# ootts/EasyHeC

Measured on AMD Instinct MI355X. Metric: mask-render fwd+bwd frames/sec, xArm7 50k-tri @1280x720x8-view, higher is better.
Workload: dtype f32; 1 GPU; xarm7_1280x720_8view; robot=xarm7 (41096 tris, 20525 verts), views_per_gpu=8, global_views=8, links=8, antialias=True, optimizer=Adam lr 3e-3 wd 5e-4, ref_sums=bound once, mask_output=False, step=HIP launch chain, parallelism=single GPU

## Files before the change

easyhec_amd/csrc/ehr_fused_core.h:

```cpp
#pragma once
#include "ehr_host.h"
#include "ehr_pose_core.h"
#include "ehr_raster_core.h"

namespace ehr {

#define EHR_FIX_SCALE 4294967296.0
__device__ __forceinline__ long long fix_of(float v) { return __double2ll_rn((double)v * EHR_FIX_SCALE); }
__device__ __forceinline__ void fix_add(long long* acc, float v, int* meta) {
    if (!(fabsf(v) < 1.0e9f)) {
        atomicOr(&meta[EHR_META_OVERFLOW], 1);
        return;
    }
    if (v != 0.f) atomicAdd((unsigned long long*)acc, (unsigned long long)fix_of(v));
}
__device__ __forceinline__ void fix_add_delta(long long* acc, float v, long long cached, int* meta) {
    if (!(fabsf(v) < 1.0e9f)) {
        atomicOr(&meta[EHR_META_OVERFLOW], 1);
        return;
    }
    const long long d = ((v != 0.f) ? fix_of(v) : 0ll) - cached;
    if (d != 0) atomicAdd((unsigned long long*)acc, (unsigned long long)d);
}
__device__ __forceinline__ float fix_get(long long q) { return (float)((double)q * (1.0 / EHR_FIX_SCALE)); }
__device__ __forceinline__ long long acc_load(const long long* p) {
    return __hip_atomic_load(p, __ATOMIC_RELAXED, __HIP_MEMORY_SCOPE_AGENT);
}

__host__ __device__ constexpr int vb_acc_stride(int L, int nls = VB_LOSS_SLOTS) { return 12 * L + nls * VB_LOSS_STRIDE; }
__host__ __device__ __forceinline__ int* vb_acc_meta(long long* acc, int B, int L) { return (int*)(acc + (size_t)B * vb_acc_stride(L)); }

struct StepTail {
    const float* K;
    const float* link_poses;
    const float* tc_jac;
    float* red;
    float* dof;
    float* m;
    float* v;
    int* step;
    float* loss_out;
    float* grad_out;
    float n, f, lr, b1, b2, eps, wd;
    int defer_adam;
};

struct FinishPre {
    AdamState st;
    PoseBwdPre pb;
    long long vt;
};

template <bool TAIL>
__device__ __forceinline__ void finish_prefetch(FinishPre& pre, const BinGeom& g, int B, const long long* __restrict__ vtot,
                                                const StepTail& tail, int nls, float (*Js)[16] ,
                                                float* lp_lds ) {
    const int tid = threadIdx.x;
    if (TAIL && !tail.defer_adam) pre.st = pose_adam_fetch(tail.dof, tail.m, tail.v, tail.step);
    pre.vt = (nls == 32 && vtot && (tid & 31) == 0 && (tid >> 5) < B) ? vtot[tid >> 5] : 0ll;
    if (TAIL) {
        pose_backward_prefetch(pre.pb, tail.K, tail.link_poses, tail.tc_jac, B, g.L, g.H, g.W, tail.n, tail.f, Js, lp_lds);
        if (!tail.defer_adam) pose_adam_bias(pre.st, tail.lr, tail.b1, tail.b2);
    }
}

template <bool TAIL>
__device__ __forceinline__ void finish_reduce(const FinishPre& pre, const BinGeom& g, int B, const long long* __restrict__ facc,
                                              const long long* __restrict__ vtot, float* __restrict__ loss,
                                              float* __restrict__ grad_mvp, int* __restrict__ meta, const StepTail& tail,
                                              int nls, int lstride, double (*S)[17] ,
                                              float* red_lds , float (*Js)[16] ,
                                              const float* lp_lds ) {
    const int tid = threadIdx.x, L = g.L;
    const int acc_stride = vb_acc_stride(L, nls);
    auto view_loss_slow = [&](int b) {
// ... 120 lines not shown
```

easyhec_amd/csrc/ehr_host.h:

```cpp
#pragma once
#include <hip/hip_runtime.h>
#include <stdint.h>
#include <stdio.h>

#include <string>
#include <vector>

#include "../../include/ehr.h"

struct ehr_ctx;

namespace ehr {

void set_error(const std::string& msg);
int fail(int code, const char* fmt, ...);

#define EHR_HIP(call)                                                                                   \
    do {                                                                                                \
        hipError_t e_ = (call);                                                                         \
        if (e_ != hipSuccess)                                                                           \
            return ::ehr::fail(EHR_ERR_HIP, "%s failed: %s (%s:%d)", #call, hipGetErrorString(e_), __FILE__, __LINE__); \
    } while (0)

#define EHR_LAUNCH_CHECK()                                                                              \
// ... 30 lines not shown
int vbuf_plan(ehr_ctx* ctx, int B, int L, int V, int T, int H, int W, float slack, const float* verts,
              const int32_t* tris, const int32_t* tri_link, const int32_t* opp);
int vbuf_meta_read(ehr_ctx* ctx, int* meta4);
int vbuf_bind_ref(ehr_ctx* ctx, const float* ref, int views, hipStream_t stream);
int vbuf_score(ehr_ctx* ctx, const float* verts, const int32_t* tris, const int32_t* vert_link, const float* mvp, int Q, int S,
               int L, int V, int T, int H, int W, long long* score, unsigned char* count, hipStream_t stream, int* handled);
int vbuf_overlap(ehr_ctx* ctx, const float* verts, const int32_t* tris, const int32_t* vert_link, const float* mvp,
                 const float* ref, int Q, int S, int L, int V, int T, int H, int W, long long* overlap, long long* ref_area,
                 hipStream_t stream, int* handled);
int vbuf_chain(ehr_ctx* ctx, const float* verts, const int32_t* tris, const int32_t* vert_link,
               const int32_t* opp, float* mvp, const float* ref, int B, int L, int V, int T, int H, int W, float* mask,
               float* loss, float* grad_mvp, const StepHead* head, const StepTail* tail, hipStream_t stream,
               int multi_views = 0);

}

struct ehr_ctx {
    int device = 0;
    ehr::Scratch counts;
    unsigned long long counts_clean = ~0ull;
    bool vb_slow_needed = false;
    ehr::Scratch ranges;
    std::vector<int32_t> ranges_last;
    unsigned long long ranges_moves = ~0ull;
    ehr::Scratch rkeys;
    unsigned long long rkeys_clean = ~0ull;
    ehr::Scratch offsets;
    ehr::Scratch entries;
    size_t entries_cap = 0;
    int* host_pinned = nullptr;
    hipEvent_t ev_size[2] = {nullptr, nullptr};
    bool size_valid[2] = {false, false};
    ehr::RasterShape size_shape[2] = {};
    int size_slot = 0;
    int pB = 0, pL = 0, pV = 0, pT = 0, pH = 0, pW = 0;
    int num_cus = 256;
    ehr::Scratch vb_clus;
    ehr::Scratch vb_heavy;
    ehr::Scratch vb_idx;
    const void* vb_plan_tris = nullptr;
    const void* vb_plan_opp = nullptr;
    const void* vb_plan_verts = nullptr;
    int vb_nc = 0;
    int vb_jcap = 0;
    int vb_chunk = 0;
    ehr::Scratch vb_boxes;
    ehr::Scratch vb_units;
    ehr::Scratch vb_acc;
    ehr::Scratch vb_posc;
    bool vb_lazy = false;
    ehr::Scratch vb_jobs;
    ehr::Scratch vb_spill;
    int vb_spill_cap = 0;
    ehr::Scratch vb_refsum;
    const float* vb_ref = nullptr;
    int vb_ref_views = 0;
    const float* vb_weight = nullptr;
    int vb_weight_views = 0;
    ehr::Scratch vb_hstate;
    ehr::Scratch vb_hstate_m;
    ehr::Scratch sc_counts, sc_offsets, sc_entries, sc_posc;
    ehr::Scratch sc_img;
    size_t sc_entries_cap = 0;
    ehr::Scratch sc_clus, sc_misc;
    int sc_nc = 0;
    const void* sc_key[3] = {nullptr, nullptr, nullptr};
    int sc_key_n[3] = {0, 0, 0};
    unsigned long long sc_hash = 0;
    bool sc_mixed = false;
    void* comm = nullptr;
    int comm_ranks = 0;
    void* p2p_mail = nullptr;
    void* p2p_peer[EHR_P2P_MAX_RANKS] = {};
    int p2p_ranks = 0, p2p_rank = 0;
    hipStream_t cap_stream = nullptr;
    hipGraphExec_t gexec = nullptr;
    unsigned long long gexec_reallocs = 0;
    unsigned long long scratch_moves() const {
        unsigned long long n = 0;
        for (const ehr::Scratch* s : {&counts, &offsets, &entries, &vb_clus, &vb_heavy, &vb_idx, &vb_boxes, &vb_units, &vb_acc,
                                      &vb_posc, &vb_jobs, &vb_spill, &vb_refsum, &vb_hstate, &vb_hstate_m, &sc_counts, &sc_offsets, &sc_entries, &sc_posc, &sc_clus, &sc_misc, &sc_img})
            n += s->moves;
        return n;
    }
    bool capturing = false;
    bool timing = false;
    std::vector<hipEvent_t> ev;
    size_t ev_used = 0;
};
```

easyhec_amd/csrc/ehr_vbuf.hip:

```cpp
#include <stdlib.h>
#include <string.h>

#include <algorithm>
#include <utility>
#include <vector>

#include "ehr_fused_core.h"

namespace ehr {

constexpr int VB_RW = EHR_TILE_W + 2;
constexpr int VB_RH = EHR_TILE_H + 2;
constexpr int VB_RN = VB_RW * VB_RH;
constexpr int VB_WORDS = (VB_RN + 63) / 64;
constexpr int VB_LBOX_STRIDE = 16;
constexpr int VB_HEAVY_T_DEFAULT = 3000;
constexpr int VB_HEAVY_CAP = 4096;
constexpr int VB_MED_CAP = 2048;
constexpr int VB_MED_T_DEFAULT = 1500;
constexpr int VB_PRIO_LONG = 3;
constexpr int VB_PRIO_HEAVY = 2;
constexpr int VB_JOB_ITEMS = 64;
constexpr int VB_SPILL_BLOCK = 2048;
constexpr u64 VB_EMPTY = ~0ull;
// ... 1445 lines not shown
        for (int j = 0; j < 4; j++)
            if (ix + j < W) mask[im + j] = 0.f;
    }
}

struct VbCompArgs {
    const long long* tsum;
    int nls, want_grad, vec_ok;
    float* loss;
    int B;
    long long* facc;
    int do_finish, B_all;
    const float* mvp;
    int spill_cap;
    int* lbox_all;
    VbSlots sl;
    float* mask;
    const float* verts;
    const float* ref;
    const long long* vtot_all;
    int* meta;
    float* grad_mvp;
    const VbItem* spill;
    int V;
    const long long* facc_all;
    const int* ref_flag;
    BinGeom g;
};

struct VbSharedRef {
    int view0, nviews;
};
struct VbWeight {
    const float* w;
    int view0, nviews;
};
struct VbCompParamsW;
typedef const VbCompParamsW __attribute__((address_space(4)))* VbCompParamsWPtr;
__device__ __forceinline__ VbCompParamsWPtr vb_comp_params_w();
__device__ __forceinline__ VbWeight vb_comp_weight(VbCompParamsWPtr p);
__device__ __forceinline__ void vb_read_weights(const VbWeight& wt, int b, int H, int W, int row, int ix, const bool* pin, int vec_ok, float* wf) {
    const size_t imw = ((size_t)((wt.view0 + b) % wt.nviews) * H + row) * W + ix;
    if (vec_ok) {
        if (pin[0]) {
            const float4 w4 = *reinterpret_cast<const float4*>(wt.w + imw);
            wf[0] = w4.x; wf[1] = w4.y; wf[2] = w4.z; wf[3] = w4.w;
        }
    } else {
#pragma unroll
        for (int j = 0; j < 4; j++)
            if (pin[j]) wf[j] = wt.w[imw + j];
    }
}
template <bool FILL, bool SHARED = false, bool WEIGHTED = false>
__device__ __forceinline__ void vb_composite_items(const VbCompArgs& C, const int* s_jbase, const unsigned* s_utile, float* gpix,
                                                   int xcd, int wslot, int nslots, int nwg, VbSharedRef sh = {0, 1}) {
    const BinGeom& g = C.g;
    const int lane = lane_id(), wave = (int)(threadIdx.x >> 6);
    const int W = g.W, H = g.H, L = g.L, B = C.B, U = B * L;
    const bool sparse = C.tsum != nullptr;
    const int jcap = C.sl.jcap, nls = C.nls, want_grad = C.want_grad, vec_ok = C.vec_ok, V = C.V, spill_cap = C.spill_cap;
    const float *const mvpc = C.mvp, *const verts = C.verts, *const jval = C.sl.jval, *const ref = C.ref;
    const int *const jn = C.sl.jn, *const jspill = C.sl.jspill;
    const VbItem *const jitems = C.sl.jitems, *const spill = C.spill;
    float* const mask = C.mask;
    long long* const facc = C.facc;
    int* const meta = C.meta;
    const long long* const tsum = C.tsum;
    const int nitems = sparse ? min(s_jbase[U], jcap) : B * g.nt;
    const int per_xcd = vb_xcd_share(nitems);
    const int ibeg = xcd * per_xcd, iend = min(ibeg + per_xcd, nitems);
    const int istep = nslots;
    const int acc_stride = vb_acc_stride(L, nls);
    const int r = lane >> 3, c4 = (lane & 7) * 4;
    const float invL = __builtin_amdgcn_rcpf((float)L);
    const VbCompParamsWPtr wparams = vb_comp_params_w();
    for (int item = ibeg + wslot; item < iend; item += istep) {
    int b, tx, ty;
    if (sparse) {
        int lo = 0;
        if (U <= 64) {
            lo = __popcll(__ballot(lane < U && s_jbase[lane] <= item)) - 1;
        } else {
            int hi = U - 1;
            while (lo < hi) {
                const int mid = (lo + hi + 1) >> 1;
                if (s_jbase[mid] <= item)
                    lo = mid;
                else
                    hi = mid - 1;
            }
        }
        b = vb_div_small(lo, invL);
        const unsigned ut = s_utile[lo];
        const int nx = (int)(ut >> 22), k = item - s_jbase[lo];
        const int kr = vb_div_small(k, __builtin_amdgcn_rcpf((float)nx));
        ty = (int)((ut >> 10) & 4095u) + kr;
        tx = (int)(ut & 1023u) + k - kr * nx;
        bool prior = false;
        if (lane < lo - b * L) {
            const int u2 = b * L + lane;
            const unsigned u2t = s_utile[u2];
            const int n2 = s_jbase[u2 + 1] - s_jbase[u2];
            const int ax0 = u2t & 1023u, ay0 = (u2t >> 10) & 4095u, anx = u2t >> 22;
            prior = n2 > 0 && tx >= ax0 && tx < ax0 + anx && ty >= ay0 && (ty - ay0) * anx < n2;
        }
        if (__ballot(prior)) continue;
    } else {
        b = item / g.nt;
        const int tile = item - b * g.nt;
        tx = tile % g.ntx;
        ty = tile / g.ntx;
    }
    const int tile = ty * g.ntx + tx;
    long long* const vacc = facc + (size_t)b * acc_stride;
    long long* const lacc = vacc + 12 * L + (tile % nls) * VB_LOSS_STRIDE;
    const int rx0 = tx * EHR_TILE_W - 1, ry0 = ty * EHR_TILE_H - 1;
    unsigned tmask;
    int myn = -1, myslot = 0;
    {
        if (lane < L) {
            const int u = b * L + lane;
            const unsigned ut = s_utile[u];
            const int j0 = s_jbase[u], n = s_jbase[u + 1] - j0;
            const int tx0 = ut & 1023u, ty0 = (ut >> 10) & 4095u, nx = ut >> 22;
            if (n > 0 && tx >= tx0 && tx < tx0 + nx && ty >= ty0 && (ty - ty0) * nx < n) {
                myslot = j0 + (ty - ty0) * nx + (tx - tx0);
                if (myslot < jcap) myn = jn[myslot];
            }
        }
        tmask = (unsigned)__ballot(myn >= 0);
    }
    if (sparse && tmask == 0) {
        if (FILL) {
            const int zx = tx * EHR_TILE_W + c4, zy = ty * EHR_TILE_H + r;
            vb_zero_tile_row(mask, ((size_t)b * H + (H - 1 - (zy < H ? zy : 0))) * W + zx, zy < H, zx, W, vec_ok);
        }
        continue;
    }
    const int ix = tx * EHR_TILE_W + c4, iy = ty * EHR_TILE_H + r;
    const bool row_in = iy < H;
    const size_t im = ((size_t)b * H + (H - 1 - (row_in ? iy : 0))) * W + ix;
    const size_t imr = SHARED ? ((size_t)((sh.view0 + b) % sh.nviews) * H + (H - 1 - (row_in ? iy : 0))) * W + ix : im;
    float rf[4] = {0.f, 0.f, 0.f, 0.f};
    bool pin[4];
#pragma unroll
    for (int j = 0; j < 4; j++) pin[j] = row_in && (ix + j) < W;
    if (vec_ok) {
        if (pin[0]) {
            const float4 r4 = *reinterpret_cast<const float4*>(ref + imr);
            rf[0] = r4.x; rf[1] = r4.y; rf[2] = r4.z; rf[3] = r4.w;
        }
    } else {
#pragma unroll
        for (int j = 0; j < 4; j++)
            if (pin[j]) rf[j] = ref[imr + j];
    }
    float wf[4] = {0.f, 0.f, 0.f, 0.f};
    if (WEIGHTED) vb_read_weights(vb_comp_weight(wparams), b, H, W, H - 1 - (row_in ? iy : 0), ix, pin, vec_ok, wf);
    float acc[4] = {0.f, 0.f, 0.f, 0.f};
    unsigned todo = tmask;
    while (todo) {
        const int l = __ffs(todo) - 1;
        todo &= todo - 1;
        const size_t slot = (size_t)vb_readlane(myslot, l);
        const float4 v4 = *reinterpret_cast<const float4*>(jval + slot * 256 + r * EHR_TILE_W + c4);
        acc[0] += v4.x;
        acc[1] += v4.y;
        acc[2] += v4.z;
        acc[3] += v4.w;
    }
    float e2 = 0.f, gv[4];
    float mv[4];
#pragma unroll
    for (int j = 0; j < 4; j++) {
        gv[j] = 0.f;
        mv[j] = 0.f;
        if (pin[j]) {
            const float m = acc[j] > 1.f ? 1.f : acc[j];
            const float e = m - rf[j];
            if (WEIGHTED) {
                const float we = wf[j] * e;
                e2 += we * e;
                gv[j] = (acc[j] <= 1.f) ? 2.f * we : 0.f;
            } else {
                e2 += e * e;
                gv[j] = (acc[j] <= 1.f) ? 2.f * e : 0.f;
            }
            mv[j] = m;
        }
    }
    if (mask) {
        if (vec_ok) {
            if (pin[0]) *reinterpret_cast<float4*>(mask + im) = make_float4(mv[0], mv[1], mv[2], mv[3]);
        } else {
#pragma unroll
            for (int j = 0; j < 4; j++)
                if (pin[j]) mask[im + j] = mv[j];
        }
    }
    {
        const float s = wave_sum(e2);
        if (lane == 0) {
            if (sparse)
                fix_add_delta(lacc, s, tsum[(size_t)b * g.nt + tile], meta);
            else
                fix_add(lacc, s, meta);
        }
    }
    const unsigned bmask = (unsigned)__ballot(myn > 0);
    if (!want_grad || bmask == 0) continue;

    VB_WAVE_SYNC();
#pragma unroll
    for (int j = 0; j < 4; j++) gpix[r * EHR_TILE_W + c4 + j] = gv[j];
    VB_WAVE_SYNC();
    unsigned links = bmask;
    while (links) {
        const int l = __ffs(links) - 1;
        links &= links - 1;
        const size_t slot = (size_t)vb_readlane(myslot, l);
        int n = vb_readlane(myn, l);
        int sbase = 0;
        if (n > VB_JOB_ITEMS) {
            sbase = jspill[slot];
            if (sbase < 0 || sbase >= spill_cap) n = VB_JOB_ITEMS;
            else n = min(n, VB_JOB_ITEMS + (spill_cap - sbase));
        }
        const VbVertsT<true> pv = vb_verts<true>(VbLazy{verts, mvpc + ((size_t)b * L + l) * 16, nullptr});
        float G[12];
#pragma unroll
        for (int k = 0; k < 12; k++) G[k] = 0.f;
        for (int i = lane; i < n; i += 64) {
            const VbItem itm = *((i < VB_JOB_ITEMS) ? &jitems[slot * VB_JOB_ITEMS + i] : &spill[sbase + (i - VB_JOB_ITEMS)]);
            const int q = itm.packed & 1023, d = (itm.packed >> 10) & 1;
            const int tri1 = (itm.packed >> 13) & 1;
            const float dc = ((itm.packed >> 14) & 1) ? 1.f : -1.f;
            const int nq = q + (d ? VB_RW : 1);
            const int oq = (itm.alpha > 0.f) ? q : nq;
            const int oy = vb_div_rw(oq), ox = oq - oy * VB_RW;
            const float gi = gpix[(oy - 1) * EHR_TILE_W + (ox - 1)];
            const float dd = gi * dc;
            if (gi == 0.f || dd == 0.f) continue;
            const int qy = vb_div_rw(q), qx = q - qy * VB_RW;
            int px = rx0 + qx, py = ry0 + qy;
            if (tri1) {
                px += 1 - d;
                py += d;
            }
            float g1[3], g2[3];
            const float* a1 = verts + 3 * (size_t)itm.v1;
            const float* a2 = verts + 3 * (size_t)itm.v2;
            const float h1[4] = {a1[0], a1[1], a1[2], 1.f}, h2[4] = {a2[0], a2[1], a2[2], 1.f};
            aa_pos_grad(transform_vertex(pv.M, h1[0], h1[1], h1[2]), transform_vertex(pv.M, h2[0], h2[1], h2[2]), px, py, d,
                        itm.alpha, dd, W, H, g1, g2);
#pragma unroll
            for (int rr = 0; rr < 3; rr++)
#pragma unroll
                for (int c = 0; c < 4; c++) G[4 * rr + c] += g1[rr] * h1[c] + g2[rr] * h2[c];
        }
        const float mine = wave_sum12(G, lane);
        if ((lane & 3) == 0 && (lane & 12) != 12) fix_add(&vacc[12 * l + wave_sum12_element(lane)], mine, meta);
    }
    }
    if (FILL) {
        const int total = B * g.nt;
        for (int t = (int)blockIdx.x * 4 + wave; t < total; t += nwg * 4) {
            const int b = t / g.nt, tile = t - b * g.nt;
            const int ty = tile / g.ntx, tx = tile - ty * g.ntx;
            bool owned = false;
            if (lane < L) {
                const int u = b * L + lane;
                const unsigned ut = s_utile[u];
                const int n = s_jbase[u + 1] - s_jbase[u];
                const int tx0 = ut & 1023u, ty0 = (ut >> 10) & 4095u, nx = ut >> 22;
                owned = n > 0 && tx >= tx0 && tx < tx0 + nx && ty >= ty0 && (ty - ty0) * nx < n;
            }
            if (__ballot(owned)) continue;
            const int ix = tx * EHR_TILE_W + c4, iy = ty * EHR_TILE_H + r;
            const bool row_in = iy < H;
            vb_zero_tile_row(mask, ((size_t)b * H + (H - 1 - (row_in ? iy : 0))) * W + ix, row_in, ix, W, vec_ok);
        }
    }
}

constexpr int VB_JOB_WAVES = 4;
struct VbCoverOut {
    u64* tcov;
    int* sticky;
    int S;
};
struct VbJobParams {
    BinGeom g;
    int B;
    VbClusters cl;
    VbRecs rc;
    const int* lbox;
    int use_hint;
    VbHeavy hv;
    VbSlotIdx si;
    int heavy_t, med_t0;
    VbResolveArgs rq;
    VbCoverOut co;
};
typedef const VbJobParams __attribute__((address_space(4)))* VbJobParamsPtr;
__device__ __forceinline__ VbJobParamsPtr vb_job_params() {
    VbJobParamsPtr p = (VbJobParamsPtr)__builtin_amdgcn_kernarg_segment_ptr();
    asm volatile("" : "+s"(p));
    return p;
}
template <class T>
__device__ __forceinline__ T vb_prm_copy(const T __attribute__((address_space(4)))* p) {
    return *(const T*)p;
}
template <bool COVER, bool LAZY = false>
// ... 343 lines not shown
    const int r = lane >> 3, c4 = (lane & 7) * 4;
    const int ix = tx * EHR_TILE_W + c4, iy = ty * EHR_TILE_H + r;
    const bool row_in = iy < H;
    const size_t im = ((size_t)b * H + (H - 1 - (row_in ? iy : 0))) * W + ix;
    float rf[4] = {0.f, 0.f, 0.f, 0.f};
    bool pin[4];
#pragma unroll
    for (int j = 0; j < 4; j++) pin[j] = row_in && (ix + j) < W;
    if (vec_ok) {
        if (pin[0]) {
            const float4 r4 = *reinterpret_cast<const float4*>(ref + im);
            rf[0] = r4.x; rf[1] = r4.y; rf[2] = r4.z; rf[3] = r4.w;
        }
    } else {
#pragma unroll
        for (int j = 0; j < 4; j++)
            if (pin[j]) rf[j] = ref[im + j];
    }
    float wf[4] = {0.f, 0.f, 0.f, 0.f};
    if (WEIGHTED) vb_read_weights(wt, b, H, W, H - 1 - (row_in ? iy : 0), ix, pin, vec_ok, wf);
    float e2 = 0.f;
#pragma unroll
    for (int j = 0; j < 4; j++)
        if (pin[j]) {
            const float e = 0.f - rf[j];
            if (WEIGHTED) {
                const float we = wf[j] * e;
                e2 += we * e;
            } else {
                e2 += e * e;
            }
        }
    const float s = wave_sum(e2);
    if (lane == 0) {
        long long q = 0;
        if (!(fabsf(s) < 1.0e9f))
            atomicOr(flag, 1);
        else if (s != 0.f)
            q = fix_of(s);
        tsum[gw] = q;
        if (q != 0) atomicAdd((unsigned long long*)&vtot[b], (unsigned long long)q);
    }
}

struct VbCompParams {
    VbCompArgs C;
    StepTail tail;
};
struct VbCompParamsW {
    VbCompArgs C;
    StepTail tail;
    VbSharedRef sh;
    VbWeight wt;
};
__device__ __forceinline__ VbCompParamsWPtr vb_comp_params_w() {
    return (VbCompParamsWPtr)__builtin_amdgcn_kernarg_segment_ptr();
}
__device__ __forceinline__ VbWeight vb_comp_weight(VbCompParamsWPtr p) {
    VbWeight wt;
    wt.w = p->wt.w;
    wt.view0 = p->wt.view0;
    wt.nviews = p->wt.nviews;
    return wt;
}
typedef const VbCompParams __attribute__((address_space(4)))* VbCompParamsPtr;
__device__ __forceinline__ VbCompParamsPtr vb_comp_params() {
    VbCompParamsPtr p = (VbCompParamsPtr)__builtin_amdgcn_kernarg_segment_ptr();
    asm volatile("" : "+s"(p));
    return p;
}

constexpr int VB_FINISH_POLLS = 1 << 21;
__device__ __forceinline__ int vb_comp_arrivals(int xcd, int per, int nitems, int nfill, int nlbox) {
    const int share = vb_xcd_share(nitems);
    const int mine = max(0, min(share, nitems - xcd * share));
    int n = (mine + 3) >> 2;
    const int fwg = (nfill + 3) >> 2, lwg = (nlbox + 255) >> 8;
    n = max(n, fwg > xcd ? vb_xcd_share(fwg - xcd) : 0);
    n = max(n, lwg > xcd ? vb_xcd_share(lwg - xcd) : 0);
    return min(n, per);
}

template <bool TAIL, bool FILL, bool SHARED = false, bool WEIGHTED = false>
__global__ void __launch_bounds__(256, FILL ? 5 : 6)
vb_composite_kernel(VbCompArgs C, StepTail tail, VbSharedRef sh, VbWeight wt) {
    __shared__ float gpix_all[4][EHR_TILE_W * EHR_TILE_H];
    extern __shared__ int s_dyn[];
    const int tid = threadIdx.x, lane = tid & 63, wave = tid >> 6;
    float* const gpix = gpix_all[wave];
    const int U = C.B * C.g.L;
    int* const s_jbase = s_dyn;
    unsigned* const s_utile = reinterpret_cast<unsigned*>(s_dyn + U + 1);
    const bool sparse = C.tsum != nullptr;
    for (int i = tid; i <= U; i += 256) s_jbase[i] = C.sl.jbase[i];
    for (int i = tid; i < U; i += 256) s_utile[i] = C.sl.jutile[i];
    if (C.do_finish && C.lbox_all)
        for (int i = (int)blockIdx.x * 256 + tid; i < VB_LBOX_STRIDE * C.B_all * C.g.L; i += (int)gridDim.x * 256)
            C.lbox_all[i] = (i & 2) ? INT_MIN : INT_MAX;
    __syncthreads();
    const int nwg = gridDim.x, xcd = blockIdx.x & (VB_XCDS - 1);
    vb_composite_items<FILL, SHARED, WEIGHTED>(C, s_jbase, s_utile, gpix, xcd, (int)(blockIdx.x >> VB_XCD_BITS) * 4 + wave, (nwg >> VB_XCD_BITS) * 4, nwg, sh);
    if (!vb_comp_params()->C.do_finish) return;
    const VbCompParamsPtr Q = vb_comp_params();
    const int per = nwg >> VB_XCD_BITS;
    const int nitems = sparse ? min(s_jbase[U], Q->C.sl.jcap) : Q->C.B * Q->C.g.nt;
    const int nfill = FILL ? Q->C.B * Q->C.g.nt : 0, nlbox = Q->C.lbox_all ? VB_LBOX_STRIDE * Q->C.B_all * Q->C.g.L : 0;
    const int kblk = (int)(blockIdx.x >> VB_XCD_BITS);
    const bool finisher = (int)blockIdx.x == nwg - VB_XCDS;
    const bool arrives = kblk < vb_comp_arrivals(xcd, per, nitems, nfill, nlbox);
    if (!finisher) {
        if (!arrives) return;
        asm volatile("s_waitcnt vmcnt(0)" ::: "memory");
        __syncthreads();
        if (tid == 0)
            (void)__hip_atomic_fetch_add(vb_line(Q->C.meta, VB_LINE_COMP_ARRIVE + xcd), 1, __ATOMIC_RELAXED, __HIP_MEMORY_SCOPE_AGENT);
        return;
    }
    __shared__ double S[4][17];
    __shared__ float red_lds[8];
    __shared__ float Js[6][16];
    const long long* const vtot = sparse ? Q->C.vtot_all : nullptr;
    const BinGeom g = ((const VbCompParams*)Q)->C.g;
    const StepTail tl = ((const VbCompParams*)Q)->tail;
    FinishPre pre;
    __syncthreads();
    finish_prefetch<TAIL>(pre, g, Q->C.B_all, vtot, tl, Q->C.nls, Js, gpix_all[0]);
    if (Q->C.ref_flag && tid == 0 && Q->C.ref_flag[0]) atomicOr(&Q->C.meta[EHR_META_OVERFLOW], 1);
    if (wave == 0) {
        int* const ctr = vb_line(Q->C.meta, VB_LINE_COMP_ARRIVE + (lane & (VB_XCDS - 1)));
        const int want = vb_comp_arrivals(lane & (VB_XCDS - 1), per, nitems, nfill, nlbox) - (((lane & (VB_XCDS - 1)) == 0 && arrives) ? 1 : 0);
        bool done = false;
        for (int polls = 0; polls < VB_FINISH_POLLS; polls++) {
            const int have = (lane < VB_XCDS) ? __hip_atomic_load(ctr, __ATOMIC_RELAXED, __HIP_MEMORY_SCOPE_AGENT) : want;
            done = __ballot(have < want) == 0;
            if (done) break;
            __builtin_amdgcn_s_sleep(2);
        }
        if (lane < VB_XCDS) __hip_atomic_store(ctr, 0, __ATOMIC_RELAXED, __HIP_MEMORY_SCOPE_AGENT);
        if (!done && lane == 0) atomicOr(&Q->C.meta[EHR_META_OVERFLOW], 1);
    }
    asm volatile("s_waitcnt vmcnt(0)" ::: "memory");
    __syncthreads();
    __builtin_amdgcn_fence(__ATOMIC_ACQUIRE, "agent");
    finish_reduce<TAIL>(pre, g, Q->C.B_all, Q->C.facc_all, vtot, Q->C.loss, Q->C.grad_mvp, Q->C.meta, tl, Q->C.nls, VB_LOSS_STRIDE, S, red_lds, Js, gpix_all[0]);
}

__global__ void __launch_bounds__(256)
vb_finish_multi_kernel(MultiFinish A, StepTail tail) {
    __shared__ double S[4][17];
    __shared__ float red_lds[8];
    __shared__ float Js[6][16];
    __shared__ float lp_lds[1024];
    const int p = blockIdx.x, tid = threadIdx.x, L = A.g.L;
    for (int i = p * 256 + tid; i < VB_LBOX_STRIDE * A.P * A.Bv * L; i += (int)gridDim.x * 256)
        A.lbox_all[i] = (i & 2) ? INT_MIN : INT_MAX;
    tail.tc_jac += 7 * 16 * p;
    tail.red += 8 * p;
    tail.dof += 6 * p;
    tail.m += 6 * p;
    tail.v += 6 * p;
    tail.step += p;
    if (tail.loss_out) tail.loss_out += p;
    if (tail.grad_out) tail.grad_out += 6 * p;
    const size_t v0 = (size_t)p * A.Bv;
    const long long* const vtot = A.vtot_all ? A.vtot_all + v0 : nullptr;
    FinishPre pre;
// ... 321 lines not shown
    cl.cvert = (const float4*)(((uintptr_t)(cl.laabb + 6 * (size_t)L) + 15) & ~(uintptr_t)15);
    cl.NC = NC;
    VbSlotIdx si;
    si.cvidx = (const int4*)(cl.cvert + 3 * (size_t)NC1 * 64);
    return {cl, si};
}

struct VbVertexGrid {
    int gx, xcd_views;
};
static VbVertexGrid vb_vertex_grid(int num_cus, int nitems, int Bk) {
    const int per_view_cap = std::max(8, (num_cus * VB_VERTEX_GRID) / std::max(Bk, 1));
    const int items_per_wg = (nitems + per_view_cap - 1) / per_view_cap;
    VbVertexGrid v;
    v.gx = std::max(1, (nitems + items_per_wg - 1) / std::max(items_per_wg, 1));
    v.xcd_views = (VB_XCD_SPLIT && (Bk % VB_XCDS) == 0) ? Bk / VB_XCDS : 0;
    return v;
}

int ehr::vbuf_plan(ehr_ctx* ctx, int B, int L, int V, int T, int H, int W, float slack, const float* verts,
                   const int32_t* tris, const int32_t* tri_link, const int32_t* opp) {
    if (H > 32760 || W > 32736)
        return fail(EHR_ERR_INVALID, "ehr_fused_plan: resolution above 32736 x 32760 (W x H) is unsupported");
    if ((V > 0 && !verts) || (T > 0 && (!tris || !tri_link || !opp)))
        return fail(EHR_ERR_INVALID, "ehr_fused_plan: the scene arrays (verts, tris, tri_link, opp) are required");
    int rc;
    if ((rc = vb_build_clusters(ctx->vb_clus, ctx->vb_nc, L, V, T, verts, tris, tri_link))) return rc;
    const int NC = std::max(ctx->vb_nc, 1);
    BinGeom gp = make_geom(H, W, L);
    const double jobs_per_view = std::max(1.0, ((slack > 0.f) ? std::min((double)L, (double)slack) : (double)L) * gp.nt);
    const double view_bytes = jobs_per_view * VB_SLOT_BYTES + (double)NC * VB_CLUSTER_REC_BYTES + (double)std::max(V, 1) * sizeof(float4) +
                              (double)L * gp.nt * sizeof(int);
    static const double budget = getenv("EHR_VB_SCRATCH_MB") ? atof(getenv("EHR_VB_SCRATCH_MB")) * 1048576.0 : 24576.0 * 1048576.0;
    int Bc = std::min(B, std::max(1, VB_MAX_UNITS / L));
    Bc = std::max(1, std::min(Bc, (int)(budget / view_bytes)));
    if (jobs_per_view * Bc > 2.0e9) return fail(EHR_ERR_INVALID, "ehr_fused_plan: views x links x tiles of a chunk exceeds 2e9");
    ctx->vb_chunk = Bc;
    if ((rc = ctx->vb_acc.reserve((size_t)B * vb_acc_stride(L) * sizeof(long long) + VB_META_BYTES))) return rc;
    {
        const char* e = getenv("EHR_VB_LAZY");
        ctx->vb_lazy = e ? atoi(e) != 0 : (double)V > 1.5 * (double)std::max(T, 1);
        if (ctx->vb_lazy != (ctx->vb_posc.ptr == nullptr) && ctx->gexec) {
            EHR_HIP(hipGraphExecDestroy(ctx->gexec));
            ctx->gexec = nullptr;
        }
        if (!ctx->vb_lazy && (rc = ctx->vb_posc.reserve((size_t)Bc * std::max(V, 1) * sizeof(float4)))) return rc;
    }
    size_t bytes;
    vb_recs(nullptr, Bc, NC, &bytes);
    if ((rc = ctx->vb_boxes.reserve(bytes))) return rc;
    {
        const char* e = getenv("EHR_VB_SPILL_ITEMS");
        ctx->vb_spill_cap = e ? std::max(0, atoi(e)) : VB_SPILL_ITEMS;
        if ((rc = ctx->vb_spill.reserve(std::max((size_t)ctx->vb_spill_cap * sizeof(VbItem), (size_t)1 << 20)))) return rc;
    }
    if ((rc = ctx->vb_units.reserve((size_t)VB_LBOX_STRIDE * B * L * sizeof(int)))) return rc;
    {
        if ((rc = ctx->vb_refsum.reserve(((size_t)B * gp.nt + B + 1) * sizeof(long long)))) return rc;
        ctx->vb_ref = nullptr;
        ctx->vb_weight = nullptr;
        ctx->vb_weight_views = 0;
    }
    ctx->vb_jcap = (int)(jobs_per_view * Bc);
    vb_slots(nullptr, (size_t)ctx->vb_jcap, (size_t)Bc * L, &bytes);
    if ((rc = ctx->vb_jobs.reserve(bytes))) return rc;
    vb_heavy(nullptr, (size_t)Bc * L * gp.nt, &bytes);
    if ((rc = ctx->vb_heavy.reserve(bytes))) return rc;
    EHR_HIP(hipMemset(ctx->vb_heavy.ptr, 0, bytes));
    if ((rc = ctx->vb_idx.reserve((size_t)2 * std::max(T, 1) * sizeof(int4)))) return rc;
    if (T > 0) {
        vb_pad_kernel<<<(T + 255) / 256, 256>>>(tris, T, (int4*)ctx->vb_idx.ptr);
        vb_pad_kernel<<<(T + 255) / 256, 256>>>(opp, T, (int4*)ctx->vb_idx.ptr + T);
        EHR_LAUNCH_CHECK();
    }
    if (!ctx->vb_hstate.ptr) {
        if ((rc = ctx->vb_hstate.reserve(16 * sizeof(int)))) return rc;
        EHR_HIP(hipMemset(ctx->vb_hstate.ptr, 0, 16 * sizeof(int)));
    }
    if (ctx->vb_hstate_m.cap < (size_t)VB_HSTATE_INTS * B * sizeof(int)) {
        if ((rc = ctx->vb_hstate_m.reserve((size_t)VB_HSTATE_INTS * B * sizeof(int)))) return rc;
        EHR_HIP(hipMemset(ctx->vb_hstate_m.ptr, 0, ctx->vb_hstate_m.cap));
    }
    ctx->vb_plan_tris = tris;
    ctx->vb_plan_opp = opp;
    ctx->vb_plan_verts = verts;
    EHR_HIP(hipMemset(ctx->vb_acc.ptr, 0, ctx->vb_acc.cap));
    std::vector<int> boxes((size_t)VB_LBOX_STRIDE * B * L);
    for (size_t i = 0; i < boxes.size(); i++) boxes[i] = (i & 2) ? INT_MIN : INT_MAX;
    EHR_HIP(hipMemcpy(ctx->vb_units.ptr, boxes.data(), boxes.size() * sizeof(int), hipMemcpyHostToDevice));
    EHR_HIP(hipDeviceSynchronize());
    return EHR_OK;
}

int ehr::vbuf_meta_read(ehr_ctx* ctx, int* meta4) {
    EHR_HIP(hipMemcpy(meta4, vb_acc_meta((long long*)ctx->vb_acc.ptr, ctx->pB, ctx->pL), 4 * sizeof(int), hipMemcpyDeviceToHost));
    return EHR_OK;
}

int ehr::vbuf_chain(ehr_ctx* ctx, const float* verts, const int32_t* tris, const int32_t* vert_link, const int32_t* opp, float* mvp, const float* ref, int B, int L, int V,
                    int T, int H, int W, float* mask, float* loss, float* grad_mvp, const StepHead* head,
                    const StepTail* tail, hipStream_t stream, int multi_views) {
    const bool multi = multi_views > 0;
    if (tris != ctx->vb_plan_tris || opp != ctx->vb_plan_opp || verts != ctx->vb_plan_verts)
        return fail(EHR_ERR_INVALID, "fused op: the scene arrays differ from the planned ones; call ehr_fused_plan again");
    BinGeom g = make_geom(H, W, L);
    long long* const facc_all = (long long*)ctx->vb_acc.ptr;
// ... 49 lines not shown
        const VbVertexGrid vg = vb_vertex_grid(ctx->num_cus, nitems, Bk);
        const dim3 vgrid(vg.gx * Bk);
        const int nacc_ints = 2 * Bk * acc_stride;
        const int role = first_chunk ? VB_ROLE_FIRST_CHUNK : VB_ROLE_LATER_CHUNK;
        if (head && multi) {
            StepHead hk = *head;
            hk.view0 = b0;
            hk.nviews = multi_views;
            vb_vertex_kernel<true, true><<<vgrid, 256, 0, stream>>>(verts, vert_link, tris, cl, hk, mvp_k, V, nvb, g, posc, recs, lbox,
                                                                   (int*)facc, nacc_ints, meta, Bk, vg.gx, vg.xcd_views, hv, role);
        } else if (head) {
            StepHead hk = *head;
            hk.link_poses = head->link_poses + (size_t)b0 * L * 16;
            vb_vertex_kernel<true><<<vgrid, 256, 0, stream>>>(verts, vert_link, tris, cl, hk, mvp_k, V, nvb, g, posc, recs, lbox,
                                                             (int*)facc, nacc_ints, meta, Bk, vg.gx, vg.xcd_views, hv, role);
        } else {
            StepHead none = {};
            vb_vertex_kernel<false><<<vgrid, 256, 0, stream>>>(verts, vert_link, tris, cl, none, mvp_k, V, nvb, g, posc, recs,
                                                              lbox, (int*)facc, nacc_ints, meta, Bk, vg.gx, vg.xcd_views, hv, role);
        }
        EHR_LAUNCH_CHECK();
        if (time_it) EHR_HIP(hipEventRecord(ev[1], stream));
        VbResolveArgs rq;
        rq.verts = verts; rq.mvp = mvp_k; rq.posc = posc; rq.V = V; rq.L = L; rq.W = W; rq.H = H;
        rq.tri4 = (const int4*)ctx->vb_idx.ptr;
        rq.opp4 = (const int4*)ctx->vb_idx.ptr + T;
        rq.T = T;
        rq.sl = sl;
        rq.spill = spill;
        rq.spill_cap = ctx->vb_spill_cap;
        rq.meta = meta;
        rq.want_grad = grad_mvp ? 1 : 0;
        VbJobParams jp = {};
        jp.g = g; jp.B = Bk; jp.cl = cl; jp.si = si; jp.rc = recs; jp.lbox = lbox; jp.hv = hv;
        jp.use_hint = Bc == B;
        jp.heavy_t = VB_HEAVY_T_DEFAULT;
        jp.med_t0 = VB_MED_T_DEFAULT;
        jp.rq = rq;
        if (lazy)
            vb_job_kernel<false, true><<<job_wgs, 256, 0, stream>>>(jp);
        else
            vb_job_kernel<false><<<job_wgs, 256, 0, stream>>>(jp);
        EHR_LAUNCH_CHECK();
        if (with_slow) {
            vb_slow_kernel<<<VB_SLOW_GRID, 256, 0, stream>>>(rq, recs, cl.NC, si.cvidx, cl.coff);
            EHR_LAUNCH_CHECK();
        }
        if (time_it) {
            for (int k = 2; k <= 4; k++) EHR_HIP(hipEventRecord(ev[k], stream));
        }
        int nwg = ctx->num_cus * VB_COMPOSITE_GRID;
        if (!sparse) nwg = std::min(nwg, (Bk * g.nt + 3) / 4);
        nwg = std::max(VB_XCDS, vb_xcd_round_up(nwg));
        const size_t dyn = (2 * (size_t)Bk * L + 1) * sizeof(int);
        const bool fill = sparse && mask_k != nullptr;
        VbCompArgs ca;
        ca.g = g; ca.B = Bk; ca.mvp = mvp_k; ca.V = V; ca.verts = verts; ca.sl = sl; ca.ref = ref_k; ca.mask = mask_k; ca.facc = facc;
        ca.nls = VB_LOSS_SLOTS; ca.want_grad = rq.want_grad; ca.vec_ok = vec_ok; ca.spill = spill; ca.spill_cap = ctx->vb_spill_cap;
        ca.meta = meta;
        ca.tsum = sparse ? tsum_all + (size_t)b0 * g.nt : nullptr;
        ca.ref_flag = ref_flag; ca.loss = loss; ca.grad_mvp = grad_mvp;
        ca.do_finish = (last_chunk && !multi) ? 1 : 0; ca.B_all = B; ca.facc_all = facc_all; ca.vtot_all = vtot_all; ca.lbox_all = lbox_all;
        const VbWeight wt = {weight, b0, weight ? ctx->vb_weight_views : 1};
#define VB_COMPOSITE_W(TAILV, FILLV, SHAREDV, tailarg, sharg)                                                      \
    do {                                                                                                             \
        if (weight)                                                                                                  \
            vb_composite_kernel<TAILV, FILLV, SHAREDV, true><<<nwg, 256, dyn, stream>>>(ca, tailarg, sharg, wt);     \
        else                                                                                                         \
            vb_composite_kernel<TAILV, FILLV, SHAREDV><<<nwg, 256, dyn, stream>>>(ca, tailarg, sharg, wt);           \
    } while (0)
#define VB_COMPOSITE(TAILV, FILLV, tailarg) VB_COMPOSITE_W(TAILV, FILLV, false, tailarg, (VbSharedRef{0, 1}))
        StepTail none = {};
        if (multi) {
            const VbSharedRef sh = {b0, multi_views};
            if (fill)
                VB_COMPOSITE_W(false, true, true, none, sh);
            else
                VB_COMPOSITE_W(false, false, true, none, sh);
        } else if (tail) {
            if (fill) VB_COMPOSITE(true, true, *tail); else VB_COMPOSITE(true, false, *tail);
        } else {
            if (fill) VB_COMPOSITE(false, true, none); else VB_COMPOSITE(false, false, none);
        }
#undef VB_COMPOSITE
#undef VB_COMPOSITE_W
        EHR_LAUNCH_CHECK();
    }
    if (ev) EHR_HIP(hipEventRecord(ev[5], stream));
    if (multi) {
        MultiFinish mf;
        mf.facc_all = facc_all; mf.vtot_all = vtot_all; mf.ref_flag = ref_flag; mf.loss = loss; mf.grad_mvp = grad_mvp;
        mf.meta = meta; mf.lbox_all = lbox_all; mf.P = B / multi_views; mf.Bv = multi_views; mf.nls = VB_LOSS_SLOTS; mf.g = g;
        vb_finish_multi_kernel<<<mf.P, 256, 0, stream>>>(mf, *tail);
        EHR_LAUNCH_CHECK();
    }
    if (ev) {
        for (int k = 6; k <= 7; k++) EHR_HIP(hipEventRecord(ev[k], stream));
    }
    return EHR_OK;
}

struct VbScoreMisc {
    int* lbox;
    int* meta;
    VbHeavy hv;
    int* sticky;
    size_t zero_bytes;
    unsigned long long* sacc;
    u64* tcov;
    void* own;
};
static VbScoreMisc vb_score_misc(void* base, size_t Qc, size_t Bc, int L, int nt, size_t own_bytes, size_t* bytes = nullptr) {
    VbCarve c{(uintptr_t)base};
    VbScoreMisc m;
    m.lbox = c.take<int>((size_t)VB_LBOX_STRIDE * Bc * L);
    m.meta = (int*)c.take<char>(VB_META_BYTES, alignof(int));
    size_t hv_bytes;
    m.hv = vb_heavy((void*)c.at, 0, &hv_bytes);
    c.at += hv_bytes;
    m.hv.stamp = m.hv.gen;
    m.sticky = c.take<int>(16);
    m.zero_bytes = c.at - (uintptr_t)m.hv.gen;
// ... 254 lines not shown
```

Baseline: 116,500 frames/s.

## Stage composite gradient/loss atomics in per-workgroup LDS table before global flush

Adds an LDS accumulation table in the composite kernel that covers up to two 'home' views per workgroup. Fixed-point gradient and loss atomics for items in those views go to shared memory and are flushed to global memory once at the end of the kernel. Other views still use global atomics. This cuts contended global 64-bit atomics, at the cost of more LDS (which may reduce occupancy), an extra barrier and flush pass, and a changed arrival handshake for non-finisher waves.

```diff
diff --git a/easyhec_amd/csrc/ehr_fused_core.h b/easyhec_amd/csrc/ehr_fused_core.h
--- a/easyhec_amd/csrc/ehr_fused_core.h
+++ b/easyhec_amd/csrc/ehr_fused_core.h
@@ -21,6 +21,29 @@
     }
     const long long d = ((v != 0.f) ? fix_of(v) : 0ll) - cached;
     if (d != 0) atomicAdd((unsigned long long*)acc, (unsigned long long)d);
+}
+__device__ __forceinline__ void fix_add_wg(unsigned long long* tab, int ent, long long* acc, float v, int* meta) {
+    if (!(fabsf(v) < 1.0e9f)) {
+        atomicOr(&meta[EHR_META_OVERFLOW], 1);
+        return;
+    }
+    if (v == 0.f) return;
+    if (ent >= 0)
+        atomicAdd(&tab[ent], (unsigned long long)fix_of(v));
+    else
+        atomicAdd((unsigned long long*)acc, (unsigned long long)fix_of(v));
+}
+__device__ __forceinline__ void fix_add_delta_wg(unsigned long long* tab, int ent, long long* acc, float v, long long cached, int* meta) {
+    if (!(fabsf(v) < 1.0e9f)) {
+        atomicOr(&meta[EHR_META_OVERFLOW], 1);
+        return;
+    }
+    const long long d = ((v != 0.f) ? fix_of(v) : 0ll) - cached;
+    if (d == 0) return;
+    if (ent >= 0)
+        atomicAdd(&tab[ent], (unsigned long long)d);
+    else
+        atomicAdd((unsigned long long*)acc, (unsigned long long)d);
 }
 __device__ __forceinline__ float fix_get(long long q) { return (float)((double)q * (1.0 / EHR_FIX_SCALE)); }
 __device__ __forceinline__ long long acc_load(const long long* p) {
diff --git a/easyhec_amd/csrc/ehr_host.h b/easyhec_amd/csrc/ehr_host.h
--- a/easyhec_amd/csrc/ehr_host.h
+++ b/easyhec_amd/csrc/ehr_host.h
@@ -106,6 +106,7 @@
     ehr::Scratch vb_jobs;
     ehr::Scratch vb_spill;
     int vb_spill_cap = 0;
+    int vb_acc_views = 0;
     ehr::Scratch vb_refsum;
     const float* vb_ref = nullptr;
     int vb_ref_views = 0;
diff --git a/easyhec_amd/csrc/ehr_vbuf.hip b/easyhec_amd/csrc/ehr_vbuf.hip
--- a/easyhec_amd/csrc/ehr_vbuf.hip
+++ b/easyhec_amd/csrc/ehr_vbuf.hip
@@ -1521,9 +1521,33 @@
             if (pin[j]) wf[j] = wt.w[imw + j];
     }
 }
+__device__ __forceinline__ int vb_item_unit(const int* s_jbase, int U, int item, int lane) {
+    int lo = 0;
+    if (U <= 64) {
+        lo = __popcll(__ballot(lane < U && s_jbase[lane] <= item)) - 1;
+    } else {
+        int hi = U - 1;
+        while (lo < hi) {
+            const int mid = (lo + hi + 1) >> 1;
+            if (s_jbase[mid] <= item)
+                lo = mid;
+            else
+                hi = mid - 1;
+        }
+    }
+    return lo;
+}
+struct VbAccTable {
+    unsigned long long* tab;
+    int home, views;
+};
+constexpr int VB_ACC_VIEWS = 2;
+constexpr int VB_ACC_TABLE_MAX_BYTES = 16384;
+__host__ __device__ constexpr int vb_comp_table_ints(int U) { return (2 * U + 1 + 1) & ~1; }
+__host__ __device__ constexpr int vb_acc_entries(int L, int nls) { return 12 * L + nls; }
 template <bool FILL, bool SHARED = false, bool WEIGHTED = false>
 __device__ __forceinline__ void vb_composite_items(const VbCompArgs& C, const int* s_jbase, const unsigned* s_utile, float* gpix,
-                                                   int xcd, int wslot, int nslots, int nwg, VbSharedRef sh = {0, 1}) {
+                                                   int xcd, int wslot, int nslots, int nwg, VbAccTable at, VbSharedRef sh = {0, 1}) {
     const BinGeom& g = C.g;
     const int lane = lane_id(), wave = (int)(threadIdx.x >> 6);
     const int W = g.W, H = g.H, L = g.L, B = C.B, U = B * L;
@@ -1544,22 +1568,11 @@
     const int r = lane >> 3, c4 = (lane & 7) * 4;
     const float invL = __builtin_amdgcn_rcpf((float)L);
     const VbCompParamsWPtr wparams = vb_comp_params_w();
+    const int aent = vb_acc_entries(L, nls);
     for (int item = ibeg + wslot; item < iend; item += istep) {
     int b, tx, ty;
     if (sparse) {
-        int lo = 0;
-        if (U <= 64) {
-            lo = __popcll(__ballot(lane < U && s_jbase[lane] <= item)) - 1;
-        } else {
-            int hi = U - 1;
-            while (lo < hi) {
-                const int mid = (lo + hi + 1) >> 1;
-                if (s_jbase[mid] <= item)
-                    lo = mid;
-                else
-                    hi = mid - 1;
-            }
-        }
+        const int lo = vb_item_unit(s_jbase, U, item, lane);
         b = vb_div_small(lo, invL);
         const unsigned ut = s_utile[lo];
         const int nx = (int)(ut >> 22), k = item - s_jbase[lo];
@@ -1607,6 +1620,7 @@
         }
         continue;
     }
+    const int ebase = ((unsigned)(b - at.home) < (unsigned)at.views) ? (b - at.home) * aent : -1;
     const int ix = tx * EHR_TILE_W + c4, iy = ty * EHR_TILE_H + r;
     const bool row_in = iy < H;
     const size_t im = ((size_t)b * H + (H - 1 - (row_in ? iy : 0))) * W + ix;
@@ -1671,10 +1685,11 @@
     {
         const float s = wave_sum(e2);
         if (lane == 0) {
+            const int le = ebase < 0 ? -1 : ebase + 12 * L + tile % nls;
             if (sparse)
-                fix_add_delta(lacc, s, tsum[(size_t)b * g.nt + tile], meta);
+                fix_add_delta_wg(at.tab, le, lacc, s, tsum[(size_t)b * g.nt + tile], meta);
             else
-                fix_add(lacc, s, meta);
+                fix_add_wg(at.tab, le, lacc, s, meta);
         }
     }
     const unsigned bmask = (unsigned)__ballot(myn > 0);
@@ -1729,7 +1744,10 @@
                 for (int c = 0; c < 4; c++) G[4 * rr + c] += g1[rr] * h1[c] + g2[rr] * h2[c];
         }
         const float mine = wave_sum12(G, lane);
-        if ((lane & 3) == 0 && (lane & 12) != 12) fix_add(&vacc[12 * l + wave_sum12_element(lane)], mine, meta);
+        if ((lane & 3) == 0 && (lane & 12) != 12) {
+            const int e = 12 * l + wave_sum12_element(lane);
+            fix_add_wg(at.tab, ebase < 0 ? -1 : ebase + e, &vacc[e], mine, meta);
+        }
     }
     }
     if (FILL) {
@@ -2179,6 +2197,7 @@
     StepTail tail;
     VbSharedRef sh;
     VbWeight wt;
+    int acc_views;
 };
 __device__ __forceinline__ VbCompParamsWPtr vb_comp_params_w() {
     return (VbCompParamsWPtr)__builtin_amdgcn_kernarg_segment_ptr();
@@ -2210,23 +2229,46 @@
 
 template <bool TAIL, bool FILL, bool SHARED = false, bool WEIGHTED = false>
 __global__ void __launch_bounds__(256, FILL ? 5 : 6)
-vb_composite_kernel(VbCompArgs C, StepTail tail, VbSharedRef sh, VbWeight wt) {
+vb_composite_kernel(VbCompArgs C, StepTail tail, VbSharedRef sh, VbWeight wt, int acc_views) {
     __shared__ float gpix_all[4][EHR_TILE_W * EHR_TILE_H];
-    extern __shared__ int s_dyn[];
+    extern __shared__ __align__(8) int s_dyn[];
     const int tid = threadIdx.x, lane = tid & 63, wave = tid >> 6;
     float* const gpix = gpix_all[wave];
     const int U = C.B * C.g.L;
     int* const s_jbase = s_dyn;
     unsigned* const s_utile = reinterpret_cast<unsigned*>(s_dyn + U + 1);
+    VbAccTable at;
+    at.tab = reinterpret_cast<unsigned long long*>(s_dyn + vb_comp_table_ints(U));
+    at.views = vb_comp_params_w()->acc_views;
     const bool sparse = C.tsum != nullptr;
     for (int i = tid; i <= U; i += 256) s_jbase[i] = C.sl.jbase[i];
     for (int i = tid; i < U; i += 256) s_utile[i] = C.sl.jutile[i];
+    for (int i = tid; i < at.views * vb_acc_entries(C.g.L, C.nls); i += 256) at.tab[i] = 0ull;
     if (C.do_finish && C.lbox_all)
         for (int i = (int)blockIdx.x * 256 + tid; i < VB_LBOX_STRIDE * C.B_all * C.g.L; i += (int)gridDim.x * 256)
             C.lbox_all[i] = (i & 2) ? INT_MIN : INT_MAX;
     __syncthreads();
     const int nwg = gridDim.x, xcd = blockIdx.x & (VB_XCDS - 1);
-    vb_composite_items<FILL, SHARED, WEIGHTED>(C, s_jbase, s_utile, gpix, xcd, (int)(blockIdx.x >> VB_XCD_BITS) * 4 + wave, (nwg >> VB_XCD_BITS) * 4, nwg, sh);
+    {
+        const int first = xcd * vb_xcd_share(sparse ? min(s_jbase[U], C.sl.jcap) : C.B * C.g.nt) + (int)(blockIdx.x >> VB_XCD_BITS) * 4;
+        at.home = min(sparse ? vb_item_unit(s_jbase, U, first, lane) / C.g.L : first / C.g.nt, C.B - 1);
+    }
+    vb_composite_items<FILL, SHARED, WEIGHTED>(C, s_jbase, s_utile, gpix, xcd, (int)(blockIdx.x >> VB_XCD_BITS) * 4 + wave, (nwg >> VB_XCD_BITS) * 4, nwg, at, sh);
+    asm volatile("s_waitcnt vmcnt(0)" ::: "memory");
+    __syncthreads();
+    if (wave == 0) {
+        const VbCompParamsPtr P = vb_comp_params();
+        const int L = P->C.g.L, nls = P->C.nls;
+        const int aent = vb_acc_entries(L, nls), n = at.views * aent;
+        long long* const facc = P->C.facc;
+        for (int i = lane; i < n; i += 64) {
+            const unsigned long long q = at.tab[i];
+            if (q != 0ull) {
+                const int vs = i / aent, e = i - vs * aent;
+                atomicAdd((unsigned long long*)(facc + (size_t)(at.home + vs) * vb_acc_stride(L, nls) + (e < 12 * L ? e : 12 * L + (e - 12 * L) * VB_LOSS_STRIDE)), q);
+            }
+        }
+    }
     if (!vb_comp_params()->C.do_finish) return;
     const VbCompParamsPtr Q = vb_comp_params();
     const int per = nwg >> VB_XCD_BITS;
@@ -2236,9 +2278,8 @@
     const bool finisher = (int)blockIdx.x == nwg - VB_XCDS;
     const bool arrives = kblk < vb_comp_arrivals(xcd, per, nitems, nfill, nlbox);
     if (!finisher) {
-        if (!arrives) return;
+        if (!arrives || wave != 0) return;
         asm volatile("s_waitcnt vmcnt(0)" ::: "memory");
-        __syncthreads();
         if (tid == 0)
             (void)__hip_atomic_fetch_add(vb_line(Q->C.meta, VB_LINE_COMP_ARRIVE + xcd), 1, __ATOMIC_RELAXED, __HIP_MEMORY_SCOPE_AGENT);
         return;
@@ -2666,6 +2707,8 @@
     {
         const char* e = getenv("EHR_VB_SPILL_ITEMS");
         ctx->vb_spill_cap = e ? std::max(0, atoi(e)) : VB_SPILL_ITEMS;
+        const char* a = getenv("EHR_VB_ACC_VIEWS");
+        ctx->vb_acc_views = a ? std::max(0, atoi(a)) : VB_ACC_VIEWS;
         if ((rc = ctx->vb_spill.reserve(std::max((size_t)ctx->vb_spill_cap * sizeof(VbItem), (size_t)1 << 20)))) return rc;
     }
     if ((rc = ctx->vb_units.reserve((size_t)VB_LBOX_STRIDE * B * L * sizeof(int)))) return rc;
@@ -2821,7 +2864,10 @@
         int nwg = ctx->num_cus * VB_COMPOSITE_GRID;
         if (!sparse) nwg = std::min(nwg, (Bk * g.nt + 3) / 4);
         nwg = std::max(VB_XCDS, vb_xcd_round_up(nwg));
-        const size_t dyn = (2 * (size_t)Bk * L + 1) * sizeof(int);
+        int accv = std::min(ctx->vb_acc_views, Bk);
+        while (accv > 0 && (size_t)accv * vb_acc_entries(L, VB_LOSS_SLOTS) * sizeof(long long) > (size_t)VB_ACC_TABLE_MAX_BYTES) accv--;
+        const size_t dyn = (size_t)vb_comp_table_ints(Bk * L) * sizeof(int) +
+                           (size_t)accv * vb_acc_entries(L, VB_LOSS_SLOTS) * sizeof(long long);
         const bool fill = sparse && mask_k != nullptr;
         VbCompArgs ca;
         ca.g = g; ca.B = Bk; ca.mvp = mvp_k; ca.V = V; ca.verts = verts; ca.sl = sl; ca.ref = ref_k; ca.mask = mask_k; ca.facc = facc;
@@ -2834,9 +2880,9 @@
 #define VB_COMPOSITE_W(TAILV, FILLV, SHAREDV, tailarg, sharg)                                                      \
     do {                                                                                                             \
         if (weight)                                                                                                  \
-            vb_composite_kernel<TAILV, FILLV, SHAREDV, true><<<nwg, 256, dyn, stream>>>(ca, tailarg, sharg, wt);     \
+            vb_composite_kernel<TAILV, FILLV, SHAREDV, true><<<nwg, 256, dyn, stream>>>(ca, tailarg, sharg, wt, accv); \
         else                                                                                                         \
-            vb_composite_kernel<TAILV, FILLV, SHAREDV><<<nwg, 256, dyn, stream>>>(ca, tailarg, sharg, wt);           \
+            vb_composite_kernel<TAILV, FILLV, SHAREDV><<<nwg, 256, dyn, stream>>>(ca, tailarg, sharg, wt, accv);     \
     } while (0)
 #define VB_COMPOSITE(TAILV, FILLV, tailarg) VB_COMPOSITE_W(TAILV, FILLV, false, tailarg, (VbSharedRef{0, 1}))
         StepTail none = {};
```

New measurement: 115,700 frames/s. Within noise of the previous version (-0.6%).
